# ChristodoulosPappas/IPLS-Java-API

Measured on AMD Instinct MI355X. Metric: aggregated-gradient GB/s (device-resident), 32 peers×4M doubles/partition, higher is better.
Workload: dtype f64

## Files before the change

ipls-java-api_amd/csrc/engine.hip:

```cpp
#include <hip/hip_runtime.h>

#include <algorithm>
#include <atomic>
#include <cstdarg>
#include <cstdio>
#include <cstdlib>
#include <cstring>
#include <deque>
#include <map>
#include <memory>
#include <mutex>
#include <new>
#include <set>
#include <string>
#include <thread>
#include <type_traits>
#include <vector>

#include "../../include/ipls_agg.h"
#include "ipls_kernels.hpp"
#include "javaser.hpp"
#include "engine.hpp"
#include "pubsub_host.hpp"
#include "reduce_plan.hpp"

using namespace ipls;
using namespace ipls::reduceplan;

namespace {

thread_local std::string g_tls_err;

constexpr int64_t kAlignElems = 32;
constexpr int kRingSlots = 4;
constexpr int kStageSlots = 3;

int64_t align_up(int64_t x, int64_t a) { return (x + a - 1) / a * a; }

struct PinnedSlot {
  void* host = nullptr;
  size_t cap = 0;
  hipEvent_t ev = nullptr;
// ... 22 lines not shown
  int device = 0;
  hipStream_t stream = nullptr;

  int64_t model_size = 0;
  int P = 0;
  int64_t chunk = 0;
  int secure = 0;
  std::vector<int64_t> len, flat_off;
  int64_t max_len = 0, flat_total = 0;
  int p_lo = 0;
  int64_t flat_base = 0;

  double* arena = nullptr;
  int64_t arena_elems = 0;
  std::vector<int64_t> agg_off, rep_off, w_off, fut_off;
  std::vector<uint8_t> agg_zero, rep_zero, fut_zero;

  PinnedSlot ring[kRingSlots];
  void* d_table[kRingSlots] = {};
  size_t d_table_cap[kRingSlots] = {};
  int ring_next = 0;
  std::vector<unsigned char> last_table;
  int last_slot = -1;

  std::mutex stage_mu;
  std::vector<ipls_stage*> stage_all, stage_idle;
  void* d_scratch = nullptr;
  size_t scratch_bytes = 0;
  hipEvent_t copy_ev = nullptr;
  static constexpr int kCopyThreads = 4;
  hipStream_t copy_stream[kCopyThreads] = {};
// ... 75 lines not shown
  if (p < 0 || p >= h->P) return fail(h, IPLS_E_RANGE, "partition %d out of range [0,%d)", p, h->P);
  return IPLS_OK;
}

int64_t target_off(ipls_dev* h, int p, int target) {
  switch (target) {
    case IPLS_TGT_AGG: return h->agg_off[p];
    case IPLS_TGT_REP: return h->rep_off[p];
    case IPLS_TGT_WEIGHTS:
    case IPLS_TGT_WADDR: return h->w_off[p];
    case IPLS_TGT_FUTURE: return h->fut_off[p];
    default: return -1;
  }
}

uint8_t* zero_flag(ipls_dev* h, int p, int target) {
  if (target == IPLS_TGT_AGG) return &h->agg_zero[p];
  if (target == IPLS_TGT_REP) return &h->rep_zero[p];
  if (target == IPLS_TGT_FUTURE) return &h->fut_zero[p];
  return nullptr;
}

int materialize(ipls_dev* h, int p, int target) {
  uint8_t* f = zero_flag(h, p, target);
  if (f && *f) {
    HIP_TRY(h, hipMemsetAsync(h->arena + target_off(h, p, target), 0, (size_t)h->len[p] * 8, h->stream));
    *f = 0;
  }
  return IPLS_OK;
}

int ensure_pinned(ipls_dev* h, PinnedSlot& s, size_t bytes) {
  if (s.pending) {
    HIP_TRY(h, hipEventSynchronize(s.ev));
    s.pending = false;
  }
  if (s.cap < bytes) {
    if (s.host) HIP_TRY(h, hipHostFree(s.host));
    s.host = nullptr;
    s.cap = 0;
    size_t cap = std::max<size_t>(bytes, 64 << 10);
    HIP_TRY(h, hipHostMalloc(&s.host, cap, hipHostMallocDefault));
// ... 400 lines not shown

int reduce_dev(ipls_dev* h, int p_first, int n_parts, const void* const* bufs, int k, Fmt fmt_in,
               int start_mode, int target, void* const* ext_dst = nullptr, bool be_out = false,
               const FinOut* fin = nullptr, bool host_src = false, const int64_t* lens = nullptr,
               bool arrival = false) {
  const bool be_in = fmt_in == kFmtBE, tr_in = fmt_trainer(fmt_in);
  auto len_of = [&](int q) -> int64_t { return lens ? lens[q] : h->len[p_first + q]; };
  auto dst_of = [&](int q) -> unsigned long long* {
    if (fin) return (unsigned long long*)(h->arena + h->w_off[p_first + q]);
    return ext_dst ? (unsigned long long*)ext_dst[q]
                   : (unsigned long long*)(h->arena + target_off(h, p_first + q, target));
  };
  if (k <= 0 && !fin) {
    if (start_mode == IPLS_START_ZERO) {
      for (int q = 0; q < n_parts; ++q) {
        uint8_t* f = ext_dst ? nullptr : zero_flag(h, p_first + q, target);
        if (f) *f = 1;
        else HIP_TRY(h, hipMemsetAsync(dst_of(q), 0, (size_t)len_of(q) * 8, h->stream));
      }
    }
    return IPLS_OK;
  }
  int start = start_mode;
  if (start_mode == IPLS_START_ACCUM && !ext_dst) {
    int nz = 0;
    for (int q = 0; q < n_parts; ++q) {
      uint8_t* f = zero_flag(h, p_first + q, target);
      nz += (f && *f) ? 1 : 0;
    }
    if (nz == n_parts) start = IPLS_START_ZERO;
    else if (nz) {
      for (int q = 0; q < n_parts; ++q) {
        int rc = materialize(h, p_first + q, target);
        if (rc) return rc;
      }
    }
  }
  if (!fin && !tr_in && n_parts == 1 && k == 1 && bufs[0]) {
    unsigned long long* d0 = dst_of(0);
    const int64_t L = len_of(0);
    if (d0 && !((uintptr_t)bufs[0] & 15) && !((uintptr_t)d0 & 15) && L > 0) {
      const auto* s0 = (const unsigned long long*)bufs[0];
      const unsigned blocks =
          std::max(1u, std::min<unsigned>(blocks_for((L >> 1), kBlock * 4), host_src ? 128u : 4096u));
      with_fold(be_in, be_out, start, [&](auto bi, auto bo, auto s) {
        hipLaunchKernelGGL((k_fold1<decltype(bi)::value, decltype(bo)::value, decltype(s)::value>), dim3(blocks),
                           dim3(kBlock), 0, h->stream, d0, s0, L);
      });
      HIP_TRY(h, hipGetLastError());
      h->last_launch = launch_info(IPLS_KERNEL_FOLD1, 0, kBlock, 4, 0, 0, blocks, be_in, be_out, start);
      if (!ext_dst)
        if (uint8_t* f = zero_flag(h, p_first, target)) *f = 0;
      return IPLS_OK;
    }
  }
  if (!fin && tr_in && arrival && !be_out && start != IPLS_START_FIRST && n_parts == 1 && k == 1 && bufs[0]) {
    unsigned long long* d0 = dst_of(0);
    const int64_t L = len_of(0);
    if (d0 && !((uintptr_t)bufs[0] & (uintptr_t)(4 * fmt_size(fmt_in) - 1)) && !((uintptr_t)d0 & 15) && L > 0) {
      const unsigned blocks = std::max(1u, std::min<unsigned>(blocks_for(L >> 2, kBlock * kFold1NarrowR), kFold1NarrowGrid));
      with_narrow(fmt_in, [&](auto s) {
        typedef decltype(s) S;
        const auto* s0 = (const typename S::elem*)bufs[0];
        with_start_za(start, [&](auto st) {
          hipLaunchKernelGGL((k_fold1_narrow<S, decltype(st)::value, kFold1NarrowR>), dim3(blocks), dim3(kBlock), 0,
                             h->stream, d0, s0, L);
        });
      });
      HIP_TRY(h, hipGetLastError());
      h->last_launch = launch_info(fmt_size(fmt_in) == 4 ? IPLS_KERNEL_FOLD1_F32 : IPLS_KERNEL_FOLD1_H16, 0, kBlock,
                                   kFold1NarrowR, 1, 0, blocks, false, false, start);
      if (!ext_dst)
        if (uint8_t* f = zero_flag(h, p_first, target)) *f = 0;
      return IPLS_OK;
    }
  }
  bool aligned16 = true;
  int64_t maxL = 0;
  for (int q = 0; q < n_parts; ++q) maxL = std::max(maxL, len_of(q));
  for (int64_t i = 0; i < (int64_t)n_parts * k; ++i) {
    if (!bufs[i]) return fail(h, IPLS_E_INVAL, "bucket pointer %lld is NULL", (long long)i);
    uintptr_t a = (uintptr_t)bufs[i];
    if (a & (uintptr_t)(fmt_size(fmt_in) - 1))
      return fail(h, IPLS_E_INVAL, "bucket %lld not %d-byte aligned", (long long)i, fmt_size(fmt_in));
    if (a & 15) aligned16 = false;
  }
  const size_t desc_bytes = sizeof(PartDesc) * n_parts;
  const size_t bytes = desc_bytes + sizeof(void*) * (size_t)n_parts * k;
  std::vector<unsigned char> tbl(bytes);
  PartDesc* pd = (PartDesc*)tbl.data();
  for (int q = 0; q < n_parts; ++q) {
    const int p = p_first + q;
    pd[q].len = len_of(q);
    pd[q].dst = dst_of(q);
    pd[q].init = pd[q].dst;
    pd[q].rep = nullptr;
    pd[q].avg = nullptr;
    if (fin) {
      pd[q].init = (const unsigned long long*)(h->arena + h->agg_off[p]);
      if (!h->rep_zero[p]) pd[q].rep = (const unsigned long long*)(h->arena + h->rep_off[p]);
      if (fin->avg)
        pd[q].avg = (unsigned long long*)((char*)fin->avg +
                                          (h->flat_off[p] - h->flat_off[p_first]) * (int64_t)fmt_size(fin->fmt));
    }
    if (!pd[q].dst) return fail(h, IPLS_E_INVAL, "destination %d is NULL", q);
    if ((uintptr_t)pd[q].dst & 7) return fail(h, IPLS_E_INVAL, "destination %d not 8-byte aligned", q);
    if ((uintptr_t)pd[q].dst & 15) aligned16 = false;
  }
  if (k > 0) std::memcpy(tbl.data() + desc_bytes, bufs, sizeof(void*) * (size_t)n_parts * k);
  void* dtab = nullptr;
  int rc = upload_table(h, tbl.data(), bytes, &dtab);
  if (rc) return rc;
  const PartDesc* dparts = (const PartDesc*)dtab;
  auto dbufs = (const unsigned long long* const*)((char*)dtab + desc_bytes);
  if (fin) {
    if (!aligned16 || (fin->avg && tr_in != fmt_trainer(fin->fmt)))
      return fail(h, IPLS_E_INVAL, "fused round needs 16-B aligned buckets and averages of the buckets' family");
    if (tr_in) {
      h->last_launch = with_narrow(fmt_in, [&](auto s) {
        typedef decltype(s) S;
        return with_narrow(fin->avg ? fin->fmt : fmt_in, [&](auto a) {
          return launch_round_narrow<S, decltype(a)>(start, h->secure, maxL, n_parts, h->stream,
                                                     (const typename S::elem* const*)dbufs, dparts, k, h->d_cnt);
        });
      });
    } else {
      h->last_launch = launch_reduce_fin(be_in, start, h->secure, maxL, n_parts, h->stream, dbufs, dparts, k, h->d_cnt);
    }
    HIP_TRY(h, hipGetLastError());
    for (int q = p_first; q < p_first + n_parts; ++q) h->agg_zero[q] = h->rep_zero[q] = 1;
    return IPLS_OK;
  }
  if (tr_in) {
    h->last_launch = with_narrow(fmt_in, [&](auto s) {
      typedef decltype(s) S;
      return launch_reduce_narrow<S>(be_out, start, aligned16, maxL, n_parts, h->stream,
                                     (const typename S::elem* const*)dbufs, dparts, k);
    });
  } else if (aligned16) {
    h->last_launch = launch_reduce(be_in, be_out, start, maxL, n_parts, h->stream, dbufs, dparts, k);
  } else {
    const ReducePlan p = plan_reduce_scalar(maxL, n_parts);
    launch_reduce_scalar(be_in, be_out, start, p, h->stream, dbufs, dparts, k);
    h->last_launch = launch_info(p, be_in, be_out, start);
  }
  HIP_TRY(h, hipGetLastError());
  if (!ext_dst)
    for (int q = 0; q < n_parts; ++q) {
      uint8_t* f = zero_flag(h, p_first + q, target);
      if (f) *f = 0;
    }
  return IPLS_OK;
}

int partition_geometry(const ipls_agg_cfg* c, std::vector<int64_t>& len, std::vector<int64_t>& off,
                       int64_t& chunk, std::string& why) {
  const int P = c->n_partitions;
  len.resize(P);
  off.resize(P);
  if (c->model_size > 0) {
    chunk = ref_chunk(c->model_size, P);
    for (int i = 0; i < P; ++i) {
      int64_t L = ((int64_t)(i + 1) * chunk > c->model_size) ? c->model_size - (int64_t)i * chunk + 1
                                                             : chunk + 1;
      if (L < 1) {
        char b[160];
// ... 65 lines not shown
    delete h;
    return fail(nullptr, rc, "%s", why.c_str());
  }
  h->len.assign(glen.begin() + p_lo, glen.begin() + p_hi);
  h->flat_off.assign(goff.begin() + p_lo, goff.begin() + p_hi);
  h->p_lo = p_lo;
  h->flat_base = p_hi > p_lo ? h->flat_off[0] : 0;
  h->P = p_hi - p_lo;
  h->device = device;
  h->model_size = cfg->model_size;
  h->secure = cfg->secure;
  h->agg_off.resize(h->P);
  h->rep_off.resize(h->P);
  h->w_off.resize(h->P);
  h->fut_off.resize(h->P);
  h->agg_zero.assign(h->P, 1);
  h->rep_zero.assign(h->P, 1);
  h->fut_zero.assign(h->P, 1);
  int64_t cur = 0;
  for (int p = 0; p < h->P; ++p) {
    h->max_len = std::max(h->max_len, h->len[p]);
    h->flat_total = std::max(h->flat_total, h->flat_off[p] + h->len[p] - 1);
    h->agg_off[p] = cur; cur = align_up(cur + h->len[p], kAlignElems);
    h->rep_off[p] = cur; cur = align_up(cur + h->len[p], kAlignElems);
    h->w_off[p] = cur;   cur = align_up(cur + h->len[p], kAlignElems);
    h->fut_off[p] = cur; cur = align_up(cur + h->len[p], kAlignElems);
  }
  h->arena_elems = cur;
  h->gbuf_len = h->model_size > 0 ? (int64_t)((int32_t)h->model_size / cfg->n_partitions) + 2 : cfg->bucket_len;
  auto cleanup = [&](int code) {
    (void)hipGetLastError();
    dev_close(h);
    return code;
// ... 356 lines not shown
  const int64_t L = h->len[p];
  if (off < 0 || n < 0 || off > L || n > L - off)
    return fail(h, IPLS_E_RANGE, "range [%lld, %lld) outside partition %d of length %lld", (long long)off,
                (long long)(off + n), p, (long long)L);
  if ((off & 1) || ((uintptr_t)src & 15))
    return fail(h, IPLS_E_INVAL, "a ranged fold needs an even start and 16-B aligned bytes");
  void* alias = nullptr;
  if (!is_pinned_host(src, &alias) || !alias)
    return fail(h, IPLS_E_INVAL, "a ranged fold reads pinned host memory (ipls_host_alloc)");
  if (n == 0) {
    *ticket = h->ticket_done;
    return IPLS_OK;
  }
  HIP_TRY(h, dev_use(h->device));
  if (int rc = materialize(h, p, target)) return rc;
  unsigned long long* d0 = (unsigned long long*)(h->arena + target_off(h, p, target)) + off;
  const auto* s0 = (const unsigned long long*)alias;
  const unsigned blocks = std::max(1u, std::min<unsigned>(blocks_for(n >> 1, kBlock * 4), 128u));
  const bool be = src_kind == IPLS_HOST_BE;
  if (be) hipLaunchKernelGGL((k_fold1<true, false, kAccum>), dim3(blocks), dim3(kBlock), 0, h->stream, d0, s0, n);
  else hipLaunchKernelGGL((k_fold1<false, false, kAccum>), dim3(blocks), dim3(kBlock), 0, h->stream, d0, s0, n);
  HIP_TRY(h, hipGetLastError());
  h->last_launch = launch_info(IPLS_KERNEL_FOLD1, 0, kBlock, 4, 0, 0, blocks, be, false, IPLS_START_ACCUM);
  *ticket = h->ticket_next++;
  return end_batch(h);
}

static int accumulate_chunked_fmt(ipls_dev* h, int p, int target, int64_t n, int src_kind, bool narrow, int64_t chunk,
                                  ipls_chunk_source source, void* ctx) {
  if (!h || !source) return fail_nl(h, IPLS_E_INVAL, "null argument");
// ... 184 lines not shown
      for (int l = 0; l < c[s].n_launches; fj += c[s].launch_len[l], ++l) {
        for (int j0 = 0; j0 < c[s].launch_len[l]; j0 += 65535) {
          const int nj = std::min(65535, c[s].launch_len[l] - j0);
          std::vector<FlatJob> jobs((size_t)nj);
          int64_t maxL = 1;
          bool all_vec = true, all_zero = true;
          for (int j = 0; j < nj; ++j) {
            const flat_job& f = fj[j0 + j];
            if (f.q < 0 || f.q >= h->P || f.ncopy < 0 || f.ncopy > h->len[f.q] - 1 || f.lo < 0)
              return fail(h, IPLS_E_INVAL, "internal: bad whole-gradient job");
            FlatJob& o = jobs[(size_t)j];
            o.lo = f.lo;
            o.ncopy = f.ncopy;
            o.L = h->len[f.q];
            o.dst = (unsigned long long*)(h->arena + h->agg_off[f.q]);
            o.zero = h->agg_zero[f.q];
            maxL = std::max(maxL, o.L);
            all_vec = all_vec && f.ncopy >= tile;
            all_zero = all_zero && o.zero;
          }
          void* djobs = nullptr;
          if (int r = upload_table(h, jobs.data(), jobs.size() * sizeof(FlatJob), &djobs)) return r;
          const dim3 grid(blocks_for(maxL, tile), (unsigned)nj);
          if (fmt == kFmtF64) launch_update_flat<FmtD64, false>(h->stream, grid, (const FlatJob*)djobs, d_in);
          else if (fmt == kFmtBE) launch_update_flat<FmtD64, true>(h->stream, grid, (const FlatJob*)djobs, d_in);
          else
            with_narrow(fmt, [&](auto sfmt) {
              launch_update_flat<decltype(sfmt), false>(h->stream, grid, (const FlatJob*)djobs, d_in);
            });
          HIP_TRY(h, hipGetLastError());
          for (int j = 0; j < nj; ++j) h->agg_zero[fj[j0 + j].q] = 0;
          h->last_launch = launch_info(IPLS_KERNEL_UPDATE_FLAT, 0, kBlock, kFlatR, all_vec ? 1 : 0, 0,
                                       (int64_t)grid.x * grid.y, fmt == kFmtBE, false, all_zero ? kZero : kAccum);
        }
      }
      return IPLS_OK;
    }();
  }
  for (int s = 0; s < n; ++s) {
    ipls_dev* h = c[s].h;
    ipls_stage* st = c[s].st;
    if (dev_use(h->device) == hipSuccess && hipEventRecord(st->free_ev, h->stream) == hipSuccess) {
      st->free_pending = true;
    } else {
      (void)hipGetLastError();
      (void)hipStreamSynchronize(h->stream);
// ... 152 lines not shown
  IPLS_LOCK(h);
  if (n_bytes < 0 || (n_bytes > 0 && !bytes)) return fail(h, IPLS_E_INVAL, "bad byte buffer");
  HIP_TRY(h, dev_use(h->device));
  bool zero_copy = false;
  if (int rc = gbuf_load(h, bytes, n_bytes, &zero_copy)) return rc;
  if (zero_copy) HIP_TRY(h, hipStreamSynchronize(h->stream));
  *gbuf = h->d_gbuf;
  *glen = h->gbuf_len;
  return IPLS_OK;
}

int dev_reset(ipls_dev* h, int p) {
  if (!h) return fail(nullptr, IPLS_E_INVAL, "null handle");
  IPLS_LOCK(h);
  if (p == IPLS_ALL_PARTITIONS) {
    for (int q = 0; q < h->P; ++q) h->agg_zero[q] = h->rep_zero[q] = 1;
    return IPLS_OK;
  }
  if (int rc = check_part(h, p)) return rc;
  h->agg_zero[p] = h->rep_zero[p] = 1;
  return IPLS_OK;
}

int dev_promote_future(ipls_dev* h, const int32_t* parts, int n_parts) {
  if (!h) return fail(nullptr, IPLS_E_INVAL, "null handle");
  IPLS_LOCK(h);
  if (n_parts < 0 || (n_parts > 0 && !parts)) return fail(h, IPLS_E_INVAL, "bad partition list");
  for (int i = 0; i < n_parts; ++i)
    if (int rc = check_part(h, parts[i])) return rc;
  for (int i = 0; i < n_parts; ++i) {
    const int p = parts[i];
    std::swap(h->agg_off[p], h->fut_off[p]);
    h->agg_zero[p] = h->fut_zero[p];
    h->fut_zero[p] = 1;
  }
  return IPLS_OK;
}

int dev_device_ptr(ipls_dev* h, int p, int target, void** ptr) {
  if (!h || !ptr) return fail(h, IPLS_E_INVAL, "null argument");
  IPLS_LOCK(h);
  if (int rc = check_part(h, p)) return rc;
  if (target_off(h, p, target) < 0) return fail(h, IPLS_E_INVAL, "bad target %d", target);
  HIP_TRY(h, dev_use(h->device));
  if (int rc = materialize(h, p, target)) return rc;
  *ptr = h->arena + target_off(h, p, target);
  return IPLS_OK;
}

int dev_read(ipls_dev* h, int p, int target, void* dst, int64_t n, int dst_kind) {
  if (!h || !dst) return fail(h, IPLS_E_INVAL, "null argument");
  IPLS_LOCK(h);
  if (int rc = check_part(h, p)) return rc;
  if (target_off(h, p, target) < 0) return fail(h, IPLS_E_INVAL, "bad target %d", target);
  const int64_t L = h->len[p];
  if (n < L) return fail(h, IPLS_E_RANGE, "output of %lld < partition length %lld", (long long)n, (long long)L);
  HIP_TRY(h, dev_use(h->device));
  if (int rc = materialize(h, p, target)) return rc;
  const double* srcd = h->arena + target_off(h, p, target);
  switch (dst_kind) {
// ... 25 lines not shown
  HIP_TRY(h, dev_use(h->device));
  if (int rc = materialize(h, p, target)) return rc;
  HIP_TRY(h, hipMemsetAsync(h->d_sum, 0, 8, h->stream));
  const int64_t L = h->len[p];
  hipLaunchKernelGGL(k_checksum<false>, dim3(std::max(1u, std::min<unsigned>(blocks_for(L, kBlock * 8), 2048))),
                     dim3(kBlock), 0, h->stream,
                     (const unsigned long long*)(h->arena + target_off(h, p, target)), L, h->d_sum);
  HIP_TRY(h, hipGetLastError());
  unsigned long long v = 0;
  if (int rc = d2h(h, &v, h->d_sum, 8)) return rc;
  *out = v;
  return IPLS_OK;
}

static int finalize_range(ipls_dev* h, int p0, int np) {
  bool rep_zero_all = true;
  for (int q = p0; q < p0 + np; ++q) {
    if (int rc = materialize(h, q, IPLS_TGT_AGG)) return rc;
    rep_zero_all = rep_zero_all && h->rep_zero[q];
  }
  if (!rep_zero_all)
    for (int q = p0; q < p0 + np; ++q)
      if (int rc = materialize(h, q, IPLS_TGT_REP)) return rc;
  std::vector<FinDesc> fd(np);
  int64_t maxL = 0;
  for (int q = 0; q < np; ++q) {
    fd[q] = FinDesc{h->len[p0 + q], h->agg_off[p0 + q], h->rep_off[p0 + q], h->w_off[p0 + q]};
    maxL = std::max(maxL, fd[q].len);
  }
  void* dtab = nullptr;
  if (int rc = upload_table(h, fd.data(), fd.size() * sizeof(FinDesc), &dtab)) return rc;
  const int64_t tile = kFinTile;
  const int tpp = (int)((maxL + tile - 1) / tile);
  if (rep_zero_all)
    hipLaunchKernelGGL((k_finalize<true, false>), dim3((unsigned)tpp * np), dim3(kBlock), 0, h->stream,
                       (const FinDesc*)dtab, h->arena, tpp);
  else
    hipLaunchKernelGGL((k_finalize<false, false>), dim3((unsigned)tpp * np), dim3(kBlock), 0, h->stream,
                       (const FinDesc*)dtab, h->arena, tpp);
  HIP_TRY(h, hipGetLastError());
  for (int q = p0; q < p0 + np; ++q) h->agg_zero[q] = h->rep_zero[q] = 1;
  return IPLS_OK;
}

static int divide_table(ipls_dev* h, int p0, int np, const DivDesc** dtab, int* tpp) {
  std::vector<DivDesc> dd(np);
  int64_t maxn = 0;
  for (int q = 0; q < np; ++q) {
    const int p = p0 + q;
    dd[q] = DivDesc{h->len[p], h->w_off[p], h->flat_off[p] - h->flat_off[p0]};
    maxn = std::max(maxn, h->len[p] - 1);
  }
  *tpp = (int)((std::max<int64_t>(maxn, 0) + kDivTile - 1) / kDivTile);
  if (*tpp == 0) return IPLS_OK;
  void* d = nullptr;
  if (int rc = upload_table(h, dd.data(), dd.size() * sizeof(DivDesc), &d)) return rc;
// ... 292 lines not shown
  for (auto& kv : h->other)
    if (kv.second.n > h->len[kv.first.first])
      return fail(h, IPLS_E_RANGE, "stored replica of %lld doubles > partition %d length %lld "
                  "(ArrayIndexOutOfBoundsException, IPLS.java:1225)", (long long)kv.second.n, kv.first.first,
                  (long long)h->len[kv.first.first]);
  if (participants)
    for (int q = 0; q < h->P; ++q) participants[q] = 0;
  int folded = 0;
  for (auto& it : seq) {
    const int p = it->first.first;
    const int64_t n = it->second.n;
    if (participants)
      participants[p] = (int32_t)((uint32_t)participants[p] + (uint32_t)it->second.received * (uint32_t)n);
    if (n > 0) {
      if (int rc = materialize(h, p, IPLS_TGT_REP)) return rc;
      auto rdst = (unsigned long long*)(h->arena + h->rep_off[p]);
      const bool vec = al16(rdst) && al16(it->second.d);
      if (vec)
        hipLaunchKernelGGL((k_fold_n<false, false, true>), ew_grid(n, true, 4096), dim3(kBlock), 0, h->stream, rdst,
                           it->second.d, n);
      else
        hipLaunchKernelGGL((k_fold_n<false, false, false>), ew_grid(n, false, 4096), dim3(kBlock), 0, h->stream,
                           rdst, it->second.d, n);
      HIP_TRY(h, hipGetLastError());
    }
    ++folded;
  }
  HIP_TRY(h, hipStreamSynchronize(h->stream));
  for (auto& kv : h->other) hipFree(kv.second.d);
  h->other.clear();
// ... 16 lines not shown
    const int64_t L = h->len[p];
    if (fmt_trainer(fmt))
      with_narrow(fmt, [&](auto s) {
        typedef decltype(s) S;
        hipLaunchKernelGGL(k_load_model_narrow<S>, dim3(blocks_for(L, kBlock)), dim3(kBlock), 0, h->stream,
                           (const typename S::elem*)d, h->flat_off[p] - h->flat_base, L - 1, L,
                           h->arena + h->w_off[p]);
      });
    else if (be)
      hipLaunchKernelGGL(k_load_model<true>, dim3(blocks_for(L, kBlock)), dim3(kBlock), 0, h->stream, d,
                         h->flat_off[p] - h->flat_base, L - 1, L, h->arena + h->w_off[p]);
    else
      hipLaunchKernelGGL(k_load_model<false>, dim3(blocks_for(L, kBlock)), dim3(kBlock), 0, h->stream, d,
                         h->flat_off[p] - h->flat_base, L - 1, L, h->arena + h->w_off[p]);
    HIP_TRY(h, hipGetLastError());
    h->agg_zero[p] = h->rep_zero[p] = h->fut_zero[p] = 1;
  }
  HIP_TRY(h, hipStreamSynchronize(h->stream));
  return IPLS_OK;
}

static int split_bounds(ipls_dev* h, int p, int64_t n, int64_t* ncopy) {
  const int64_t lo = h->flat_off[p];
  const int64_t hi = std::min(lo + h->chunk, n);
  const int64_t nc = std::max<int64_t>(0, hi - lo);
  if (nc > h->len[p] - 1)
    return fail(h, IPLS_E_RANGE, "gradient vector of %lld values overruns partition %d (ArrayIndexOutOfBounds, IPLS.java:1030)",
                (long long)n, p);
  *ncopy = nc;
  return IPLS_OK;
}
// ... 93 lines not shown
    const char* base = (const char*)flat + esz * h->flat_base;
    for (int i = 0; i < n_owned; ++i) {
      const int64_t lo = h->flat_off[owned[i]] - h->flat_base;
      if (nc[owned[i]] > 0)
        if (int rc = stage_h2d(h, (char*)h->d_scratch + esz * lo, base + esz * lo, (size_t)nc[owned[i]] * esz)) return rc;
    }
    d = (const unsigned long long*)h->d_scratch;
    be = src_kind == IPLS_HOST_BE;
  } else if (int rc = flat_to_device(h, (const char*)flat + esz * h->flat_base, seg, src_kind, &d, &be)) {
    return rc;
  }
  for (int i = 0; i < n_owned; ++i) {
    const int p = owned[i];
    const int64_t L = h->len[p];
    unsigned long long* acc = (unsigned long long*)(h->arena + h->agg_off[p]);
    const bool zero = h->agg_zero[p];
    const int64_t lo = h->flat_off[p] - h->flat_base;
    const bool vec = al16((const char*)d + esz * lo) && al16(acc);
    const dim3 g = vec ? dim3(std::max(1u, blocks_for(L, kEwTile))) : dim3(blocks_for(L, kBlock));
    auto flags = [&](auto&& f) {
      with_bool(zero, [&](auto z) { with_bool(vec, [&](auto v) { f(z, v); }); });
    };
    if (fmt_trainer(fmt))
      with_narrow(fmt, [&](auto s) {
        typedef decltype(s) S;
        flags([&](auto z, auto v) {
          hipLaunchKernelGGL((k_split_narrow<S, false, decltype(z)::value ? 2 : 1, decltype(v)::value>), g,
                             dim3(kBlock), 0, h->stream, (const typename S::elem*)d, lo, nc[p], L, acc);
        });
      });
    else
      with_bool(be, [&](auto bi) {
        flags([&](auto z, auto v) {
          hipLaunchKernelGGL((k_split<decltype(bi)::value, false, decltype(z)::value ? 2 : 1, decltype(v)::value>), g,
                             dim3(kBlock), 0, h->stream, d, lo, nc[p], L, acc);
        });
      });
    HIP_TRY(h, hipGetLastError());
    h->agg_zero[p] = 0;
  }
  return IPLS_OK;
}

int dev_get_partitions(ipls_dev* h, void* out, int64_t n, int out_kind) {
  if (!h || !out) return fail(h, IPLS_E_INVAL, "null argument");
  IPLS_LOCK(h);
  const int64_t M = h->flat_total - h->flat_base;
  if (n < M) return fail(h, IPLS_E_RANGE, "output of %lld < model size %lld", (long long)n, (long long)M);
  if (out_kind != IPLS_HOST_F64 && out_kind != IPLS_HOST_BE_CANON && out_kind != IPLS_DEV_F64 &&
      !kind_trainer(out_kind))
    return fail(h, IPLS_E_INVAL, "bad out_kind %d", out_kind);
  HIP_TRY(h, dev_use(h->device));
  if (kind_trainer(out_kind)) {
    const Fmt fmt = kind_fmt(out_kind);
// ... 372 lines not shown
    n = nd;
    src_kind = IPLS_HOST_BE;
  }
  if (n < L) return fail(h, IPLS_E_RANGE, "bucket of %lld doubles shorter than partition length %lld", (long long)n, (long long)L);
  HIP_TRY(h, dev_use(h->device));
  const void* d = src;
  bool be = src_kind == IPLS_HOST_BE || src_kind == IPLS_DEV_BE;
  if (src_kind == IPLS_HOST_F64 || src_kind == IPLS_HOST_BE) {
    if (int rc = ensure_scratch(h, (size_t)L * 8)) return rc;
    if (int rc = stage_h2d(h, h->d_scratch, src, (size_t)L * 8)) return rc;
    d = h->d_scratch;
  } else if (src_kind != IPLS_DEV_F64 && src_kind != IPLS_DEV_BE) {
    return fail(h, IPLS_E_INVAL, "bad src_kind %d", src_kind);
  }
  if (int rc = materialize(h, p, target)) return rc;
  double* t = h->arena + target_off(h, p, target);
  const bool vec = al16(t) && al16(d);
  const dim3 g = ew_grid(L, vec, 8192);
  auto gs = (const unsigned long long*)d;
  if (be) {
    if (vec) hipLaunchKernelGGL((k_blend<true, true>), g, dim3(kBlock), 0, h->stream, t, gs, L, a, b);
    else hipLaunchKernelGGL((k_blend<true, false>), g, dim3(kBlock), 0, h->stream, t, gs, L, a, b);
  } else {
    if (vec) hipLaunchKernelGGL((k_blend<false, true>), g, dim3(kBlock), 0, h->stream, t, gs, L, a, b);
    else hipLaunchKernelGGL((k_blend<false, false>), g, dim3(kBlock), 0, h->stream, t, gs, L, a, b);
  }
  HIP_TRY(h, hipGetLastError());
  return IPLS_OK;
}

int dev_scale(ipls_dev* h, int p, int dst_target, int src_target, double c) {
  if (!h) return fail(nullptr, IPLS_E_INVAL, "null handle");
  IPLS_LOCK(h);
  if (int rc = check_part(h, p)) return rc;
  if (target_off(h, p, dst_target) < 0 || target_off(h, p, src_target) < 0) return fail(h, IPLS_E_INVAL, "bad target");
  HIP_TRY(h, dev_use(h->device));
  if (int rc = materialize(h, p, src_target)) return rc;
  if (uint8_t* f = zero_flag(h, p, dst_target)) *f = 0;
  const int64_t L = h->len[p];
  double* sd = h->arena + target_off(h, p, dst_target);
  auto ss = (const double*)(h->arena + target_off(h, p, src_target));
  if (al16(sd) && al16(ss))
    hipLaunchKernelGGL(k_scale<true>, ew_grid(L, true, 8192), dim3(kBlock), 0, h->stream, sd, ss, L, c);
  else
    hipLaunchKernelGGL(k_scale<false>, ew_grid(L, false, 8192), dim3(kBlock), 0, h->stream, sd, ss, L, c);
  HIP_TRY(h, hipGetLastError());
  return IPLS_OK;
}

int ipls_encode_secure(const void* src, void* dst, int64_t n, int src_kind, int dst_kind, void* stream) {
  if (!src || !dst || n < 0) return fail(nullptr, IPLS_E_INVAL, "bad argument");
  if ((src_kind != IPLS_DEV_F64 && src_kind != IPLS_DEV_BE) || (dst_kind != IPLS_DEV_F64 && dst_kind != IPLS_DEV_BE))
    return fail(nullptr, IPLS_E_INVAL, "device operands only (DEV_F64 / DEV_BE)");
// ... 213 lines not shown
  }
  out[o++] = 0x78;
  return o;
}

int64_t dev_commit_partial(ipls_dev* h, int p, int32_t workers, uint8_t* out, int64_t out_cap) {
  if (!h) return fail(nullptr, IPLS_E_INVAL, "null handle");
  IPLS_LOCK(h);
  if (int rc = check_part(h, p)) return rc;
  const int64_t L = h->len[p];
  const int64_t hl = javaser::pair_header_len(), total = hl + 8 * L + javaser::pair_trailer_len();
  if (!out) return total;
  if (out_cap < total) return fail(h, IPLS_E_RANGE, "partial update needs %lld bytes", (long long)total);
  HIP_TRY(h, dev_use(h->device));
  javaser::write_pair_header(out, workers, (int32_t)L);
  if (h->agg_zero[p]) {
    std::memset(out + hl, 0, (size_t)L * 8);
  } else {
    if (int rc = ensure_scratch(h, (size_t)L * 8)) return rc;
    launch_bswap(h->stream, (const unsigned long long*)(h->arena + h->agg_off[p]), (unsigned long long*)h->d_scratch, L);
    HIP_TRY(h, hipGetLastError());
    if (int rc = d2h(h, out + hl, h->d_scratch, (size_t)L * 8)) return rc;
  }
  javaser::write_pair_trailer(out + hl + 8 * L);
  return total;
}

int64_t dev_merge_files(ipls_dev* h, const uint8_t* const* files, const int64_t* lens, int k, int file_kind,
                             uint8_t* out, int64_t out_cap) {
  if (!h) return fail(nullptr, IPLS_E_INVAL, "null handle");
  IPLS_LOCK(h);
// ... 102 lines not shown
  HIP_TRY(h, dev_use(h->device));
  FrameEnc fe{};
  const uint32_t hv[3] = {(uint32_t)n, (uint32_t)a, (uint32_t)b};
  fe.hdr[0] = (unsigned char)((uint16_t)pid >> 8);
  fe.hdr[1] = (unsigned char)pid;
  for (int f = 0; f < 3; ++f)
    for (int i = 0; i < 4; ++i) fe.hdr[2 + 4 * f + i] = (unsigned char)(hv[f] >> (24 - 8 * i));
  fe.n = n;
  fe.origin_len = origin_len;
  fe.origin = nullptr;
  if (origin_len > 0) {
    void* d = nullptr;
    if (int rc = upload_table(h, origin, (size_t)origin_len, &d)) return rc;
    fe.origin = (const unsigned char*)d;
  }
  uint8_t* zf = zero_flag(h, p, target);
  const unsigned long long* src =
      (zf && *zf) ? nullptr : (const unsigned long long*)(h->arena + target_off(h, p, target));
  unsigned char* dst = (unsigned char*)out;
  if (out_kind == IPLS_DEV_TEXT && !kernel_writable(out))
    return fail(h, IPLS_E_INVAL, "DEV_TEXT output is neither device memory nor pinned host memory");
  const bool dev_direct = out_kind == IPLS_DEV_TEXT && !((uintptr_t)out & 15);
  if (!dev_direct) {
    if (int rc = ensure_scratch(h, (size_t)T + 64)) return rc;
    dst = (unsigned char*)h->d_scratch;
  }
  const int64_t groups = (F + 23) / 24;
  hipLaunchKernelGGL(k_b64url_encode_frame, dim3(std::max(1u, std::min<unsigned>(blocks_for(groups, kBlock), 16384))),
                     dim3(kBlock), 0, h->stream, fe, src, dst, groups, T);
  HIP_TRY(h, hipGetLastError());
  if (out_kind == IPLS_DEV_TEXT) {
    if (!dev_direct) HIP_TRY(h, hipMemcpyAsync(out, dst, (size_t)T, hipMemcpyDeviceToDevice, h->stream));
    return T;
// ... 36 lines not shown
  std::vector<FrameJob> jobs(n);
  int64_t max_groups = 1;
  for (int i = 0; i < n; ++i) {
    const int p = parts[i];
    FrameJob& j = jobs[i];
    j = FrameJob{};
    const int64_t L = h->len[p];
    const uint32_t hv[3] = {(uint32_t)L, (uint32_t)a, (uint32_t)b[i]};
    j.f.hdr[0] = (unsigned char)((uint16_t)pid >> 8);
    j.f.hdr[1] = (unsigned char)pid;
    for (int f = 0; f < 3; ++f)
      for (int k = 0; k < 4; ++k) j.f.hdr[2 + 4 * f + k] = (unsigned char)(hv[f] >> (24 - 8 * k));
    j.f.n = L;
    j.f.origin_len = origin_len;
    j.f.origin = dorig;
    uint8_t* zf = zero_flag(h, p, target);
    j.src = (zf && *zf) ? nullptr : (const unsigned long long*)(h->arena + target_off(h, p, target));
    j.out = base + offs[i];
    j.groups = (14 + 8 * L + origin_len + 23) / 24;
    j.text_len = lens[i];
    max_groups = std::max(max_groups, j.groups);
  }
  void* djobs = nullptr;
  if (int rc = upload_table(h, jobs.data(), jobs.size() * sizeof(FrameJob), &djobs)) return rc;
  const unsigned gx = std::max(1u, std::min<unsigned>(blocks_for(max_groups, kBlock), 16384));
  hipLaunchKernelGGL(k_b64url_encode_frames, dim3(gx, (unsigned)n), dim3(kBlock), 0, h->stream,
                     (const FrameJob*)djobs);
  HIP_TRY(h, hipGetLastError());
  if (direct) return IPLS_OK;
  const hipMemcpyKind kind = out_kind == IPLS_DEV_TEXT ? hipMemcpyDeviceToDevice : hipMemcpyDeviceToHost;
  for (int i = 0; i < n; ++i)
    HIP_TRY(h, hipMemcpyAsync((unsigned char*)out + offs[i], base + offs[i], (size_t)lens[i], kind, h->stream));
// ... 22 lines not shown
    j.suffix = e.suffix;
    std::memcpy(j.prefix, e.prefix, (size_t)e.prefix_len);
    const int64_t body = boxed ? 14 * j.n - 6 : 8 * j.n;
    total += e.prefix_len + body + (e.suffix >= 0 ? 1 : 0);
    max_words = std::max(max_words, body / 16 + 1);
  }
  HIP_TRY_NL(h, dev_use(h->device));
  ipls_stage* st = nullptr;
  if (int rc = stage_acquire(h, (size_t)total + 32, (size_t)std::max<int64_t>(16, std::min(slot_bytes, total)), &st))
    return rc;
  int rc = IPLS_OK;
  {
    std::lock_guard<std::mutex> lk(h->mu);
    rc = flush_pending(h);
    for (int i = 0; i < n && !rc; ++i) {
      const uint8_t* zf = zero_flag(h, entries[i].q, target);
      jobs[(size_t)i].src =
          (zf && *zf) ? nullptr : (const unsigned long long*)(h->arena + target_off(h, entries[i].q, target));
    }
    void* djobs = nullptr;
    if (!rc) rc = upload_table(h, jobs.data(), jobs.size() * sizeof(SerPackJob), &djobs);
    if (!rc) {
      const dim3 grid(std::max(1u, std::min<unsigned>(blocks_for(max_words, kSerTileWords), 16384)), (unsigned)n);
      if (boxed) hipLaunchKernelGGL(k_ser_pack_boxed, grid, dim3(kBlock), 0, h->stream, (const SerPackJob*)djobs, (unsigned char*)st->d);
      else hipLaunchKernelGGL(k_ser_pack, grid, dim3(kBlock), 0, h->stream, (const SerPackJob*)djobs, (unsigned char*)st->d);
      hipError_t e = hipGetLastError();
      if (e == hipSuccess) e = hipEventRecord(st->ready, h->stream);
      if (e != hipSuccess) {
        (void)hipGetLastError();
        rc = fail(h, IPLS_E_DEVICE, "saved-model pack: %s", hipGetErrorString(e));
      }
    }
  }
// ... 25 lines not shown
  IPLS_LOCK(h);
  std::vector<SerApplyJob> jobs((size_t)n);
  int64_t max_pairs = 1;
  for (int i = 0; i < n; ++i) {
    if (int rc = check_part(h, q[i])) return rc;
    if (target_off(h, q[i], target) < 0) return fail(h, IPLS_E_INVAL, "bad target %d", target);
    const int64_t L = h->len[q[i]];
    if (offs[i] < lo || offs[i] + 8 * L > hi) return fail(h, IPLS_E_RANGE, "payload of partition %d outside the file", q[i]);
    jobs[(size_t)i] = SerApplyJob{h->arena + target_off(h, q[i], target), L, offs[i] - lo};
    max_pairs = std::max(max_pairs, L / 2 + 1);
  }
  HIP_TRY(h, dev_use(h->device));
  if (int rc = ensure_scratch(h, (size_t)(hi - lo) + 32)) return rc;
  if (int rc = stage_h2d(h, h->d_scratch, bytes + lo, (size_t)(hi - lo))) return rc;
  for (int i = 0; i < n; ++i) {
    if (mode == IPLS_SAVED_BLEND) {
      if (int rc = materialize(h, q[i], target)) return rc;
    } else if (uint8_t* zf = zero_flag(h, q[i], target)) {
      *zf = 0;
    }
  }
  void* djobs = nullptr;
  if (int rc = upload_table(h, jobs.data(), jobs.size() * sizeof(SerApplyJob), &djobs)) return rc;
  const dim3 grid(std::max(1u, std::min<unsigned>(blocks_for(max_pairs, kSerTileWords), 16384)), (unsigned)n);
  if (mode == IPLS_SAVED_BLEND)
    hipLaunchKernelGGL(k_ser_apply<true>, grid, dim3(kBlock), 0, h->stream, (const SerApplyJob*)djobs,
                       (const unsigned char*)h->d_scratch, a, b);
  else
    hipLaunchKernelGGL(k_ser_apply<false>, grid, dim3(kBlock), 0, h->stream, (const SerApplyJob*)djobs,
                       (const unsigned char*)h->d_scratch, a, b);
  HIP_TRY(h, hipGetLastError());
  return IPLS_OK;
}

int dev_load_dlist(ipls_dev* h, const uint8_t* bytes, int64_t nvals, int64_t hi, bool apply) {
// ... 11 lines not shown
  unsigned* dflag = (unsigned*)(base + flag_off);
  if (int rc = stage_h2d(h, base, bytes + javaser::kDlistFirst - 6 + 14 * g0, (size_t)img)) return rc;
  HIP_TRY(h, hipMemsetAsync(dflag, 0, 4, h->stream));
  hipLaunchKernelGGL(k_ser_unbox, dim3(std::max(1u, std::min<unsigned>(blocks_for(hi - g0, kBlock), 8192))), dim3(kBlock), 0,
                     h->stream, (const unsigned char*)base, (int64_t)0, g0, hi, vals, dflag);
  HIP_TRY(h, hipGetLastError());
  unsigned flag = 0;
  if (int rc = d2h(h, &flag, dflag, 4)) return rc;
  if (flag) return fail(h, IPLS_E_FORMAT, "serialised ArrayList<Double>: an element is not a Double");
  if (!apply) return IPLS_OK;
  for (int p = 0; p < h->P; ++p) {
    const int64_t L = h->len[p];
    hipLaunchKernelGGL(k_load_model<false>, dim3(blocks_for(L, kBlock)), dim3(kBlock), 0, h->stream, vals,
                       h->flat_off[p] - h->flat_base, L - 1, L, h->arena + h->w_off[p]);
    HIP_TRY(h, hipGetLastError());
    h->agg_zero[p] = h->rep_zero[p] = h->fut_zero[p] = 1;
  }
  HIP_TRY(h, hipStreamSynchronize(h->stream));
  return IPLS_OK;
}

int dev_device(const ipls_dev* h) { return h ? h->device : -1; }

int dev_last_launch(const ipls_dev* h, ipls_launch_info* out) {
  if (!h || !out) return IPLS_E_INVAL;
  *out = h->last_launch;
  return IPLS_OK;
}

int dev_reduce_ext(ipls_dev* h, int n, const int64_t* lens, const void* const* bufs, int k, bool be_in,
                   int start_mode, void* const* dst) {
// ... 17 lines not shown
```

Measured before the change: 7151.

## Track accumulator state and swap buffers instead of running finalize kernel

Replaces the per-partition zero flags with a small state record (zero, clean, exposed) and uses it in finalize. When only one of the aggregate or replica buffers holds data and that buffer was produced by a from-zero fold and never handed out, finalize swaps arena offsets with the weights buffer instead of launching a copy kernel. When both are zero it only memsets the weights. This removes a full read and write pass over each partition on the common path, at the cost of more state bookkeeping that must stay correct, and it can be disabled through an environment variable.

```diff
diff --git a/ipls-java-api_amd/csrc/acc_state.hpp b/ipls-java-api_amd/csrc/acc_state.hpp
--- /dev/null
+++ b/ipls-java-api_amd/csrc/acc_state.hpp
@@ -0,0 +1,65 @@
+#pragma once
+
+#include <stdint.h>
+
+namespace ipls {
+namespace accstate {
+
+struct AccState {
+  uint8_t zero = 1;
+  uint8_t clean = 0;
+  uint8_t exposed = 0;
+};
+
+inline bool is_clean(const AccState& a) { return !a.zero && a.clean && !a.exposed; }
+
+inline void set_zero(AccState& a) { a.zero = 1; }
+
+inline void materialized(AccState& a) {
+  a.zero = 0;
+  a.clean = 1;
+}
+
+inline void fold_from_zero(AccState& a) {
+  a.zero = 0;
+  a.clean = 1;
+  a.exposed = 0;
+}
+
+inline void added_into(AccState& a) { a.zero = 0; }
+
+inline void overwritten(AccState& a) {
+  a.zero = 0;
+  a.clean = 0;
+}
+
+inline void handed_out(AccState& a) { a.exposed = 1; }
+
+inline void promote(AccState& agg, AccState& fut) {
+  agg = fut;
+  fut = AccState{};
+}
+
+inline void folded(AccState& a, int start) {
+  if (start == 1) fold_from_zero(a);
+  else if (start == 0) added_into(a);
+  else overwritten(a);
+}
+
+enum FinAction : int {
+  kKernel = 0,
+  kSwapAgg = 1,
+  kSwapRep = 2,
+  kZeroW = 3,
+};
+
+inline FinAction decide(const AccState& agg, const AccState& rep, bool allow_swap = true) {
+  if (!allow_swap) return kKernel;
+  if (agg.zero && rep.zero) return kZeroW;
+  if (rep.zero && is_clean(agg)) return kSwapAgg;
+  if (agg.zero && is_clean(rep)) return kSwapRep;
+  return kKernel;
+}
+
+}
+}
diff --git a/ipls-java-api_amd/csrc/engine.hip b/ipls-java-api_amd/csrc/engine.hip
--- a/ipls-java-api_amd/csrc/engine.hip
+++ b/ipls-java-api_amd/csrc/engine.hip
@@ -23,9 +23,11 @@
 #include "engine.hpp"
 #include "pubsub_host.hpp"
 #include "reduce_plan.hpp"
+#include "acc_state.hpp"
 
 using namespace ipls;
 using namespace ipls::reduceplan;
+using namespace ipls::accstate;
 
 namespace {
 
@@ -78,7 +80,8 @@
   double* arena = nullptr;
   int64_t arena_elems = 0;
   std::vector<int64_t> agg_off, rep_off, w_off, fut_off;
-  std::vector<uint8_t> agg_zero, rep_zero, fut_zero;
+  std::vector<AccState> agg_st, rep_st, fut_st;
+  bool fin_swap = true;
 
   PinnedSlot ring[kRingSlots];
   void* d_table[kRingSlots] = {};
@@ -184,18 +187,23 @@
   }
 }
 
-uint8_t* zero_flag(ipls_dev* h, int p, int target) {
-  if (target == IPLS_TGT_AGG) return &h->agg_zero[p];
-  if (target == IPLS_TGT_REP) return &h->rep_zero[p];
-  if (target == IPLS_TGT_FUTURE) return &h->fut_zero[p];
+AccState* acc_state(ipls_dev* h, int p, int target) {
+  if (target == IPLS_TGT_AGG) return &h->agg_st[p];
+  if (target == IPLS_TGT_REP) return &h->rep_st[p];
+  if (target == IPLS_TGT_FUTURE) return &h->fut_st[p];
   return nullptr;
 }
 
+bool logically_zero(ipls_dev* h, int p, int target) {
+  const AccState* a = acc_state(h, p, target);
+  return a && a->zero;
+}
+
 int materialize(ipls_dev* h, int p, int target) {
-  uint8_t* f = zero_flag(h, p, target);
-  if (f && *f) {
+  AccState* a = acc_state(h, p, target);
+  if (a && a->zero) {
     HIP_TRY(h, hipMemsetAsync(h->arena + target_off(h, p, target), 0, (size_t)h->len[p] * 8, h->stream));
-    *f = 0;
+    materialized(*a);
   }
   return IPLS_OK;
 }
@@ -626,8 +634,8 @@
   if (k <= 0 && !fin) {
     if (start_mode == IPLS_START_ZERO) {
       for (int q = 0; q < n_parts; ++q) {
-        uint8_t* f = ext_dst ? nullptr : zero_flag(h, p_first + q, target);
-        if (f) *f = 1;
+        AccState* a = ext_dst ? nullptr : acc_state(h, p_first + q, target);
+        if (a) set_zero(*a);
         else HIP_TRY(h, hipMemsetAsync(dst_of(q), 0, (size_t)len_of(q) * 8, h->stream));
       }
     }
@@ -636,10 +644,7 @@
   int start = start_mode;
   if (start_mode == IPLS_START_ACCUM && !ext_dst) {
     int nz = 0;
-    for (int q = 0; q < n_parts; ++q) {
-      uint8_t* f = zero_flag(h, p_first + q, target);
-      nz += (f && *f) ? 1 : 0;
-    }
+    for (int q = 0; q < n_parts; ++q) nz += logically_zero(h, p_first + q, target) ? 1 : 0;
     if (nz == n_parts) start = IPLS_START_ZERO;
     else if (nz) {
       for (int q = 0; q < n_parts; ++q) {
@@ -648,6 +653,10 @@
       }
     }
   }
+  auto note_fold = [&](int q) {
+    if (ext_dst) return;
+    if (AccState* a = acc_state(h, p_first + q, target)) folded(*a, start);
+  };
   if (!fin && !tr_in && n_parts == 1 && k == 1 && bufs[0]) {
     unsigned long long* d0 = dst_of(0);
     const int64_t L = len_of(0);
@@ -661,8 +670,7 @@
       });
       HIP_TRY(h, hipGetLastError());
       h->last_launch = launch_info(IPLS_KERNEL_FOLD1, 0, kBlock, 4, 0, 0, blocks, be_in, be_out, start);
-      if (!ext_dst)
-        if (uint8_t* f = zero_flag(h, p_first, target)) *f = 0;
+      note_fold(0);
       return IPLS_OK;
     }
   }
@@ -682,8 +690,7 @@
       HIP_TRY(h, hipGetLastError());
       h->last_launch = launch_info(fmt_size(fmt_in) == 4 ? IPLS_KERNEL_FOLD1_F32 : IPLS_KERNEL_FOLD1_H16, 0, kBlock,
                                    kFold1NarrowR, 1, 0, blocks, false, false, start);
-      if (!ext_dst)
-        if (uint8_t* f = zero_flag(h, p_first, target)) *f = 0;
+      note_fold(0);
       return IPLS_OK;
     }
   }
@@ -710,7 +717,7 @@
     pd[q].avg = nullptr;
     if (fin) {
       pd[q].init = (const unsigned long long*)(h->arena + h->agg_off[p]);
-      if (!h->rep_zero[p]) pd[q].rep = (const unsigned long long*)(h->arena + h->rep_off[p]);
+      if (!h->rep_st[p].zero) pd[q].rep = (const unsigned long long*)(h->arena + h->rep_off[p]);
       if (fin->avg)
         pd[q].avg = (unsigned long long*)((char*)fin->avg +
                                           (h->flat_off[p] - h->flat_off[p_first]) * (int64_t)fmt_size(fin->fmt));
@@ -740,7 +747,10 @@
       h->last_launch = launch_reduce_fin(be_in, start, h->secure, maxL, n_parts, h->stream, dbufs, dparts, k, h->d_cnt);
     }
     HIP_TRY(h, hipGetLastError());
-    for (int q = p_first; q < p_first + n_parts; ++q) h->agg_zero[q] = h->rep_zero[q] = 1;
+    for (int q = p_first; q < p_first + n_parts; ++q) {
+      set_zero(h->agg_st[q]);
+      set_zero(h->rep_st[q]);
+    }
     return IPLS_OK;
   }
   if (tr_in) {
@@ -757,11 +767,7 @@
     h->last_launch = launch_info(p, be_in, be_out, start);
   }
   HIP_TRY(h, hipGetLastError());
-  if (!ext_dst)
-    for (int q = 0; q < n_parts; ++q) {
-      uint8_t* f = zero_flag(h, p_first + q, target);
-      if (f) *f = 0;
-    }
+  for (int q = 0; q < n_parts; ++q) note_fold(q);
   return IPLS_OK;
 }
 
@@ -857,9 +863,13 @@
   h->rep_off.resize(h->P);
   h->w_off.resize(h->P);
   h->fut_off.resize(h->P);
-  h->agg_zero.assign(h->P, 1);
-  h->rep_zero.assign(h->P, 1);
-  h->fut_zero.assign(h->P, 1);
+  h->agg_st.assign(h->P, AccState{});
+  h->rep_st.assign(h->P, AccState{});
+  h->fut_st.assign(h->P, AccState{});
+  {
+    const char* e = std::getenv("IPLS_FINALIZE_SWAP");
+    h->fin_swap = !(e && e[0] == '0');
+  }
   int64_t cur = 0;
   for (int p = 0; p < h->P; ++p) {
     h->max_len = std::max(h->max_len, h->len[p]);
@@ -1246,6 +1256,7 @@
   }
   HIP_TRY(h, dev_use(h->device));
   if (int rc = materialize(h, p, target)) return rc;
+  if (AccState* a = acc_state(h, p, target)) added_into(*a);
   unsigned long long* d0 = (unsigned long long*)(h->arena + target_off(h, p, target)) + off;
   const auto* s0 = (const unsigned long long*)alias;
   const unsigned blocks = std::max(1u, std::min<unsigned>(blocks_for(n >> 1, kBlock * 4), 128u));
@@ -1460,7 +1471,7 @@
             o.ncopy = f.ncopy;
             o.L = h->len[f.q];
             o.dst = (unsigned long long*)(h->arena + h->agg_off[f.q]);
-            o.zero = h->agg_zero[f.q];
+            o.zero = h->agg_st[f.q].zero;
             maxL = std::max(maxL, o.L);
             all_vec = all_vec && f.ncopy >= tile;
             all_zero = all_zero && o.zero;
@@ -1475,7 +1486,11 @@
               launch_update_flat<decltype(sfmt), false>(h->stream, grid, (const FlatJob*)djobs, d_in);
             });
           HIP_TRY(h, hipGetLastError());
-          for (int j = 0; j < nj; ++j) h->agg_zero[fj[j0 + j].q] = 0;
+          for (int j = 0; j < nj; ++j) {
+            AccState& a = h->agg_st[fj[j0 + j].q];
+            if (a.zero) fold_from_zero(a);
+            else added_into(a);
+          }
           h->last_launch = launch_info(IPLS_KERNEL_UPDATE_FLAT, 0, kBlock, kFlatR, all_vec ? 1 : 0, 0,
                                        (int64_t)grid.x * grid.y, fmt == kFmtBE, false, all_zero ? kZero : kAccum);
         }
@@ -1658,11 +1673,15 @@
   if (!h) return fail(nullptr, IPLS_E_INVAL, "null handle");
   IPLS_LOCK(h);
   if (p == IPLS_ALL_PARTITIONS) {
-    for (int q = 0; q < h->P; ++q) h->agg_zero[q] = h->rep_zero[q] = 1;
+    for (int q = 0; q < h->P; ++q) {
+      set_zero(h->agg_st[q]);
+      set_zero(h->rep_st[q]);
+    }
     return IPLS_OK;
   }
   if (int rc = check_part(h, p)) return rc;
-  h->agg_zero[p] = h->rep_zero[p] = 1;
+  set_zero(h->agg_st[p]);
+  set_zero(h->rep_st[p]);
   return IPLS_OK;
 }
 
@@ -1675,8 +1694,7 @@
   for (int i = 0; i < n_parts; ++i) {
     const int p = parts[i];
     std::swap(h->agg_off[p], h->fut_off[p]);
-    h->agg_zero[p] = h->fut_zero[p];
-    h->fut_zero[p] = 1;
+    promote(h->agg_st[p], h->fut_st[p]);
   }
   return IPLS_OK;
 }
@@ -1688,6 +1706,7 @@
   if (target_off(h, p, target) < 0) return fail(h, IPLS_E_INVAL, "bad target %d", target);
   HIP_TRY(h, dev_use(h->device));
   if (int rc = materialize(h, p, target)) return rc;
+  if (AccState* a = acc_state(h, p, target)) handed_out(*a);
   *ptr = h->arena + target_off(h, p, target);
   return IPLS_OK;
 }
@@ -1743,32 +1762,56 @@
 }
 
 static int finalize_range(ipls_dev* h, int p0, int np) {
-  bool rep_zero_all = true;
+  std::vector<int> todo;
   for (int q = p0; q < p0 + np; ++q) {
-    if (int rc = materialize(h, q, IPLS_TGT_AGG)) return rc;
-    rep_zero_all = rep_zero_all && h->rep_zero[q];
-  }
-  if (!rep_zero_all)
-    for (int q = p0; q < p0 + np; ++q)
-      if (int rc = materialize(h, q, IPLS_TGT_REP)) return rc;
-  std::vector<FinDesc> fd(np);
-  int64_t maxL = 0;
-  for (int q = 0; q < np; ++q) {
-    fd[q] = FinDesc{h->len[p0 + q], h->agg_off[p0 + q], h->rep_off[p0 + q], h->w_off[p0 + q]};
-    maxL = std::max(maxL, fd[q].len);
-  }
-  void* dtab = nullptr;
-  if (int rc = upload_table(h, fd.data(), fd.size() * sizeof(FinDesc), &dtab)) return rc;
-  const int64_t tile = kFinTile;
-  const int tpp = (int)((maxL + tile - 1) / tile);
-  if (rep_zero_all)
-    hipLaunchKernelGGL((k_finalize<true, false>), dim3((unsigned)tpp * np), dim3(kBlock), 0, h->stream,
-                       (const FinDesc*)dtab, h->arena, tpp);
-  else
-    hipLaunchKernelGGL((k_finalize<false, false>), dim3((unsigned)tpp * np), dim3(kBlock), 0, h->stream,
-                       (const FinDesc*)dtab, h->arena, tpp);
-  HIP_TRY(h, hipGetLastError());
-  for (int q = p0; q < p0 + np; ++q) h->agg_zero[q] = h->rep_zero[q] = 1;
+    switch (decide(h->agg_st[q], h->rep_st[q], h->fin_swap)) {
+      case kSwapAgg:
+        std::swap(h->agg_off[q], h->w_off[q]);
+        set_zero(h->agg_st[q]);
+        break;
+      case kSwapRep:
+        std::swap(h->rep_off[q], h->w_off[q]);
+        set_zero(h->rep_st[q]);
+        break;
+      case kZeroW:
+        HIP_TRY(h, hipMemsetAsync(h->arena + h->w_off[q], 0, (size_t)h->len[q] * 8, h->stream));
+        break;
+      case kKernel: todo.push_back(q); break;
+    }
+  }
+  if (!todo.empty()) {
+    bool rep_zero_all = true;
+    for (int q : todo) {
+      if (int rc = materialize(h, q, IPLS_TGT_AGG)) return rc;
+      rep_zero_all = rep_zero_all && h->rep_st[q].zero;
+    }
+    if (!rep_zero_all)
+      for (int q : todo)
+        if (int rc = materialize(h, q, IPLS_TGT_REP)) return rc;
+    const int nk = (int)todo.size();
+    std::vector<FinDesc> fd(nk);
+    int64_t maxL = 0;
+    for (int i = 0; i < nk; ++i) {
+      const int q = todo[i];
+      fd[i] = FinDesc{h->len[q], h->agg_off[q], h->rep_off[q], h->w_off[q]};
+      maxL = std::max(maxL, fd[i].len);
+    }
+    void* dtab = nullptr;
+    if (int rc = upload_table(h, fd.data(), fd.size() * sizeof(FinDesc), &dtab)) return rc;
+    const int64_t tile = kFinTile;
+    const int tpp = (int)((maxL + tile - 1) / tile);
+    if (rep_zero_all)
+      hipLaunchKernelGGL((k_finalize<true, false>), dim3((unsigned)tpp * nk), dim3(kBlock), 0, h->stream,
+                         (const FinDesc*)dtab, h->arena, tpp);
+    else
+      hipLaunchKernelGGL((k_finalize<false, false>), dim3((unsigned)tpp * nk), dim3(kBlock), 0, h->stream,
+                         (const FinDesc*)dtab, h->arena, tpp);
+    HIP_TRY(h, hipGetLastError());
+  }
+  for (int q = p0; q < p0 + np; ++q) {
+    set_zero(h->agg_st[q]);
+    set_zero(h->rep_st[q]);
+  }
   return IPLS_OK;
 }
 
@@ -2091,6 +2134,7 @@
       participants[p] = (int32_t)((uint32_t)participants[p] + (uint32_t)it->second.received * (uint32_t)n);
     if (n > 0) {
       if (int rc = materialize(h, p, IPLS_TGT_REP)) return rc;
+      added_into(h->rep_st[p]);
       auto rdst = (unsigned long long*)(h->arena + h->rep_off[p]);
       const bool vec = al16(rdst) && al16(it->second.d);
       if (vec)
@@ -2137,7 +2181,7 @@
       hipLaunchKernelGGL(k_load_model<false>, dim3(blocks_for(L, kBlock)), dim3(kBlock), 0, h->stream, d,
                          h->flat_off[p] - h->flat_base, L - 1, L, h->arena + h->w_off[p]);
     HIP_TRY(h, hipGetLastError());
-    h->agg_zero[p] = h->rep_zero[p] = h->fut_zero[p] = 1;
+    set_zero(h->agg_st[p]), set_zero(h->rep_st[p]), set_zero(h->fut_st[p]);
   }
   HIP_TRY(h, hipStreamSynchronize(h->stream));
   return IPLS_OK;
@@ -2261,7 +2305,7 @@
     const int p = owned[i];
     const int64_t L = h->len[p];
     unsigned long long* acc = (unsigned long long*)(h->arena + h->agg_off[p]);
-    const bool zero = h->agg_zero[p];
+    const bool zero = h->agg_st[p].zero;
     const int64_t lo = h->flat_off[p] - h->flat_base;
     const bool vec = al16((const char*)d + esz * lo) && al16(acc);
     const dim3 g = vec ? dim3(std::max(1u, blocks_for(L, kEwTile))) : dim3(blocks_for(L, kBlock));
@@ -2284,7 +2328,8 @@
         });
       });
     HIP_TRY(h, hipGetLastError());
-    h->agg_zero[p] = 0;
+    if (zero) fold_from_zero(h->agg_st[p]);
+    else added_into(h->agg_st[p]);
   }
   return IPLS_OK;
 }
@@ -2687,6 +2732,7 @@
     return fail(h, IPLS_E_INVAL, "bad src_kind %d", src_kind);
   }
   if (int rc = materialize(h, p, target)) return rc;
+  if (AccState* s = acc_state(h, p, target)) overwritten(*s);
   double* t = h->arena + target_off(h, p, target);
   const bool vec = al16(t) && al16(d);
   const dim3 g = ew_grid(L, vec, 8192);
@@ -2709,7 +2755,7 @@
   if (target_off(h, p, dst_target) < 0 || target_off(h, p, src_target) < 0) return fail(h, IPLS_E_INVAL, "bad target");
   HIP_TRY(h, dev_use(h->device));
   if (int rc = materialize(h, p, src_target)) return rc;
-  if (uint8_t* f = zero_flag(h, p, dst_target)) *f = 0;
+  if (AccState* s = acc_state(h, p, dst_target)) overwritten(*s);
   const int64_t L = h->len[p];
   double* sd = h->arena + target_off(h, p, dst_target);
   auto ss = (const double*)(h->arena + target_off(h, p, src_target));
@@ -2953,7 +2999,7 @@
   if (out_cap < total) return fail(h, IPLS_E_RANGE, "partial update needs %lld bytes", (long long)total);
   HIP_TRY(h, dev_use(h->device));
   javaser::write_pair_header(out, workers, (int32_t)L);
-  if (h->agg_zero[p]) {
+  if (h->agg_st[p].zero) {
     std::memset(out + hl, 0, (size_t)L * 8);
   } else {
     if (int rc = ensure_scratch(h, (size_t)L * 8)) return rc;
@@ -3086,9 +3132,8 @@
     if (int rc = upload_table(h, origin, (size_t)origin_len, &d)) return rc;
     fe.origin = (const unsigned char*)d;
   }
-  uint8_t* zf = zero_flag(h, p, target);
   const unsigned long long* src =
-      (zf && *zf) ? nullptr : (const unsigned long long*)(h->arena + target_off(h, p, target));
+      logically_zero(h, p, target) ? nullptr : (const unsigned long long*)(h->arena + target_off(h, p, target));
   unsigned char* dst = (unsigned char*)out;
   if (out_kind == IPLS_DEV_TEXT && !kernel_writable(out))
     return fail(h, IPLS_E_INVAL, "DEV_TEXT output is neither device memory nor pinned host memory");
@@ -3155,8 +3200,7 @@
     j.f.n = L;
     j.f.origin_len = origin_len;
     j.f.origin = dorig;
-    uint8_t* zf = zero_flag(h, p, target);
-    j.src = (zf && *zf) ? nullptr : (const unsigned long long*)(h->arena + target_off(h, p, target));
+    j.src = logically_zero(h, p, target) ? nullptr : (const unsigned long long*)(h->arena + target_off(h, p, target));
     j.out = base + offs[i];
     j.groups = (14 + 8 * L + origin_len + 23) / 24;
     j.text_len = lens[i];
@@ -3209,9 +3253,9 @@
     std::lock_guard<std::mutex> lk(h->mu);
     rc = flush_pending(h);
     for (int i = 0; i < n && !rc; ++i) {
-      const uint8_t* zf = zero_flag(h, entries[i].q, target);
-      jobs[(size_t)i].src =
-          (zf && *zf) ? nullptr : (const unsigned long long*)(h->arena + target_off(h, entries[i].q, target));
+      jobs[(size_t)i].src = logically_zero(h, entries[i].q, target)
+                                ? nullptr
+                                : (const unsigned long long*)(h->arena + target_off(h, entries[i].q, target));
     }
     void* djobs = nullptr;
     if (!rc) rc = upload_table(h, jobs.data(), jobs.size() * sizeof(SerPackJob), &djobs);
@@ -3267,11 +3311,9 @@
   if (int rc = ensure_scratch(h, (size_t)(hi - lo) + 32)) return rc;
   if (int rc = stage_h2d(h, h->d_scratch, bytes + lo, (size_t)(hi - lo))) return rc;
   for (int i = 0; i < n; ++i) {
-    if (mode == IPLS_SAVED_BLEND) {
+    if (mode == IPLS_SAVED_BLEND)
       if (int rc = materialize(h, q[i], target)) return rc;
-    } else if (uint8_t* zf = zero_flag(h, q[i], target)) {
-      *zf = 0;
-    }
+    if (AccState* s = acc_state(h, q[i], target)) overwritten(*s);
   }
   void* djobs = nullptr;
   if (int rc = upload_table(h, jobs.data(), jobs.size() * sizeof(SerApplyJob), &djobs)) return rc;
@@ -3313,7 +3355,7 @@
     hipLaunchKernelGGL(k_load_model<false>, dim3(blocks_for(L, kBlock)), dim3(kBlock), 0, h->stream, vals,
                        h->flat_off[p] - h->flat_base, L - 1, L, h->arena + h->w_off[p]);
     HIP_TRY(h, hipGetLastError());
-    h->agg_zero[p] = h->rep_zero[p] = h->fut_zero[p] = 1;
+    set_zero(h->agg_st[p]), set_zero(h->rep_st[p]), set_zero(h->fut_st[p]);
   }
   HIP_TRY(h, hipStreamSynchronize(h->stream));
   return IPLS_OK;
```

After: 7140. No clear change (-0.2%).
